# taylor-santos/RelativityPathTracer

Hardware: AMD Instinct MI355X
Metric: Mrays/s (primary rays) on Scenes/bunny.txt at 3840x2160 (higher is better)
Workload: dtype f32

## Files before the change

relativitypathtracer_amd/csrc/rpt_api.hip:

```cpp
#include <hip/hip_runtime.h>

#include <cmath>
#include <cstdio>
#include <chrono>
#include <cstdlib>
#include <cstring>
#include <algorithm>
#include <atomic>
#include <functional>
#include <map>
#include <memory>
#include <mutex>
#include <string>
#include <utility>
#include <vector>

#include "../../include/rpt.h"
#include "rpt_kernels.hip.h"
#include "rpt_octree_build.hip.h"
#include "rpt_screen_bounds.hpp"
#include "rpt_bounds_certify.hpp"
#include "rpt_tile_bitmap.hpp"
#include "rpt_sky_split.hpp"
#include "rpt_workers.hpp"
// ... 909 lines not shown
    a.claim_set = (int)(ctx->claim_epoch++ & 1u);
    unsigned int *claims = (unsigned int *)ctx->claim_counters.ptr;
    const long long want = (band + sky + 3) / 4;
    static const int wgs_per_cu = std::getenv("RPT_WGS_PER_CU") ? std::atoi(std::getenv("RPT_WGS_PER_CU")) : 5;
    const unsigned int wgs = (unsigned int)std::max(1ll, std::min((long long)ctx->cu_count * wgs_per_cu, want));
    switch (v) {
    case 60: hipLaunchKernelGGL(rptd::rpt_render_kernel_persistent_w5, dim3(wgs), dim3(256), 0, ctx->stream, a, a.out16, a.plane, a.debug_rgb, claims); break;
    case 62: hipLaunchKernelGGL(rptd::rpt_render_kernel_persistent_direct_w5, dim3(wgs), dim3(256), 0, ctx->stream, a, a.out16, a.plane, a.debug_rgb, claims); break;
    case 63: hipLaunchKernelGGL(rptd::rpt_render_kernel_persistent_classic_w5, dim3(wgs), dim3(256), 0, ctx->stream, a, a.out16, a.plane, a.debug_rgb, claims); break;
    default: return fail(ctx, RPT_ERR_ARG, "unknown persistent kernel variant");
    }
    return RPT_OK;
}
#endif

#ifdef RPT_DIAGNOSTICS
#define RPT_LAUNCH_X(N) case N: hipLaunchKernelGGL(rptd::rpt_render_kernel_x##N, grid, dim3(256), 0, ctx->stream, a); break;
void launch_sky_fill(rpt_ctx *ctx, const rptd::KernelArgs &a, int tiles, const int box[4]);
int launch_diagnostic(rpt_ctx *ctx, rptd::KernelArgs &a, dim3 grid, int tiles, int v) {
    if (v == 143 || v == 2573 || (v >= 256 && v < 1000 && (v & 8))) set_band_first(ctx, a, tiles);
    switch (v) {
    case 26: {
        const int tiles_x = ((ctx->width + 31) / 32) * 4;
        const int n_tiles = tiles_x * tiles;
        if (int rc = reserve(ctx, ctx->tile_masks, (size_t)n_tiles * 8)) return rc;
        a.mask_tiles_x = tiles_x;
        a.n_tiles = n_tiles;
        a.tile_masks = (unsigned long long *)ctx->tile_masks.ptr;
        hipLaunchKernelGGL(rptd::rpt_tile_bin_kernel, dim3((n_tiles + 255) / 256), dim3(256), 0, ctx->stream, a);
        hipLaunchKernelGGL(rptd::rpt_render_kernel_v1_masked_w5, grid, dim3(256), 0, ctx->stream, a);
        break;
    }
    case 40: hipLaunchKernelGGL(rptd::rpt_render_kernel_ballot_w4, dim3(grid.x * 4, grid.y), dim3(64), 0, ctx->stream, a); break;
    case 42: hipLaunchKernelGGL(rptd::rpt_render_kernel_ballot_w6, dim3(grid.x * 4, grid.y), dim3(64), 0, ctx->stream, a); break;
    case 141: hipLaunchKernelGGL(rptd::rpt_render_kernel_r02walk_w5, grid, dim3(256), 0, ctx->stream, a); break;
    case 143: hipLaunchKernelGGL(rptd::rpt_render_kernel_r02walk_first_w5, grid, dim3(256), 0, ctx->stream, a); break;
    case 60: case 62: case 63: {
        const int rc = launch_persistent(ctx, a, tiles, v);
        if (rc > 0) return rc;
        if (rc < 0) hipLaunchKernelGGL(rptd::rpt_render_kernel_ballot_w5, dim3(grid.x * 4, grid.y), dim3(64), 0, ctx->stream, a);
        break;
    }
    case 61: hipLaunchKernelGGL(rptd::rpt_render_kernel_queue_w5, grid, dim3(256), 0, ctx->stream, a); break;
    RPT_LAUNCH_X(256) RPT_LAUNCH_X(257) RPT_LAUNCH_X(259) RPT_LAUNCH_X(261) RPT_LAUNCH_X(263) RPT_LAUNCH_X(265) RPT_LAUNCH_X(269)
    RPT_LAUNCH_X(273) RPT_LAUNCH_X(277) RPT_LAUNCH_X(285) RPT_LAUNCH_X(305) RPT_LAUNCH_X(317) RPT_LAUNCH_X(337) RPT_LAUNCH_X(349) RPT_LAUNCH_X(401) RPT_LAUNCH_X(785) RPT_LAUNCH_X(529) RPT_LAUNCH_X(541) RPT_LAUNCH_X(561) RPT_LAUNCH_X(573) RPT_LAUNCH_X(621) RPT_LAUNCH_X(641) RPT_LAUNCH_X(653)
    case 1257: hipLaunchKernelGGL(rptd::rpt_render_kernel_x257_w6, grid, dim3(256), 0, ctx->stream, a); break;
    case 2257: hipLaunchKernelGGL(rptd::rpt_render_kernel_x257_w4, grid, dim3(256), 0, ctx->stream, a); break;
    case 2259: hipLaunchKernelGGL(rptd::rpt_render_kernel_x259_w4, grid, dim3(256), 0, ctx->stream, a); break;
    case 2263: hipLaunchKernelGGL(rptd::rpt_render_kernel_x263_w4, grid, dim3(256), 0, ctx->stream, a); break;
    RPT_LAUNCH_X(689) RPT_LAUNCH_X(701)
    case 2573: hipLaunchKernelGGL(rptd::rpt_render_kernel_x573_w4, grid, dim3(256), 0, ctx->stream, a); break;
    case 7:
        if (int rc = reserve(ctx, ctx->counters, 16 * sizeof(unsigned long long))) return rc;
        RPT_HIP(ctx, hipMemsetAsync(ctx->counters.ptr, 0, 16 * sizeof(unsigned long long), ctx->stream));
        a.counters = (unsigned long long *)ctx->counters.ptr;
        hipLaunchKernelGGL(rptd::rpt_render_kernel_v1_diag, grid, dim3(256), 0, ctx->stream, a);
        break;
    case 8: hipLaunchKernelGGL(rptd::rpt_render_kernel_primary_only, grid, dim3(256), 0, ctx->stream, a); break;
    case 786: {
        if (!a.out16) return fail(ctx, RPT_ERR_ARG, "variant 786 writes the 16-byte framebuffer only");
        const int no_box[4] = {0, 0, 0, 0};
        launch_sky_fill(ctx, a, tiles, no_box);
        break;
    }
    case 11:
        if (int rc = reserve(ctx, ctx->wave_times, (size_t)grid.x * grid.y * 4 * 10 * sizeof(unsigned long long))) return rc;
        RPT_HIP(ctx, hipMemsetAsync(ctx->wave_times.ptr, 0, ctx->wave_times.bytes, ctx->stream));
// ... 2819 lines not shown
```

relativitypathtracer_amd/csrc/rpt_diag_kernels.hip.h:

```cpp
#pragma once

namespace rptd {

RPT_DEV f3 cull_dir(const DObj &o, f3 nd) {
    return mk3(o.B[0] * nd.x + o.B[1] * nd.y + o.B[2] * nd.z + o.b[0],
               o.B[3] * nd.x + o.B[4] * nd.y + o.B[5] * nd.z + o.b[1],
               o.B[6] * nd.x + o.B[7] * nd.y + o.B[8] * nd.z + o.b[2]);
}

__global__ __launch_bounds__(256) void rpt_tile_bin_kernel(const KernelArgs a) {
    const int tile = blockIdx.x * 256 + threadIdx.x;
    const bool valid = tile < a.n_tiles;
    unsigned long long mask = 0;
    if (valid) {
        const int tx = tile % a.mask_tiles_x, trow = tile / a.mask_tiles_x;
        const float x0 = (float)(tx * 8);
        const float y0 = (float)(((trow >> a.run_log2) * a.tile_step + a.first_tile + (trow & ((1 << a.run_log2) - 1))) * RPT_TILE_ROWS);
        const float xs[5] = {x0 + 3.5f, x0 - 0.5f, x0 + 7.5f, x0 - 0.5f, x0 + 7.5f};
        const float ys[5] = {y0 + 3.5f, y0 - 0.5f, y0 - 0.5f, y0 + 7.5f, y0 + 7.5f};
        f3 nd[5];
        for (int k = 0; k < 5; k++) {
            const f3 p = mk3((xs[k] / (float)a.width - 0.5f) * a.aspect, ys[k] / (float)a.height - 0.5f, 0.5f);
            nd[k] = p * (1.0f / __builtin_sqrtf(dot(p, p)));
        }
// ... 22 lines not shown
                const float thTile = 1.05f * sTile;
                const f3 to = mk3(o.cbx - o.ox, o.cby - o.oy, o.cbz - o.oz);
                const float dist = __builtin_sqrtf(dot(to, to));
                const bool sane = tile_ok && (sTile < 0.2f) && (lmin > 0.05f * lmax) && (lmax < 1.0e30f) && (dist > 1.05f * o.rb) && (dist < 1.0e30f);
                if (sane) {
                    const f3 ca = cross(u[0], to);
                    const float sinAng = __builtin_sqrtf(dot(ca, ca)) / dist;
                    const float angLow = dot(u[0], to) > 0.0f ? sinAng : 1.0f;
                    const float xs_ = o.rb / dist;
                    const float thObj = xs_ < 0.45f ? 1.05f * xs_ : asinf(fminf(xs_, 1.0f));
                    keep = !(angLow > thObj + 1.5f * thTile + 1.0e-4f);
                }
            }
            if (keep) mask |= 1ull << i;
        }
        if (a.object_count > 64) mask |= 0ull;
        a.tile_masks[tile] = mask;
    }
}


template <int N> struct DiagPolicy : KernelPolicy {
    static constexpr bool culled = N >= 20;
    static constexpr bool band_first = N == 123 || (N >= 256 && N < 1000 && (N & 8));
    static constexpr bool one_wave = false;
    static constexpr int diag = N;
};

__global__ __launch_bounds__(256) void rpt_render_kernel_v1_diag(const KernelArgs a) { render_pixel_body<DiagPolicy<2>>(a); }
__global__ __launch_bounds__(256) __attribute__((amdgpu_waves_per_eu(4, 4))) void rpt_render_kernel_v1_timeline(const KernelArgs a) { render_pixel_body<DiagPolicy<4>>(a); }
__global__ __launch_bounds__(256) void rpt_render_kernel_primary_only(const KernelArgs a) { render_pixel_body<DiagPolicy<5>>(a); }
__global__ __launch_bounds__(256) __attribute__((amdgpu_waves_per_eu(5, 5))) void rpt_render_kernel_v1_masked_w5(const KernelArgs a) { render_pixel_body<DiagPolicy<10>>(a); }
__global__ __launch_bounds__(64) __attribute__((amdgpu_waves_per_eu(4, 4))) void rpt_render_kernel_ballot_w4(const KernelArgs a) { render_pixel_body<Ballot>(a); }
__global__ __launch_bounds__(64) __attribute__((amdgpu_waves_per_eu(6, 6))) void rpt_render_kernel_ballot_w6(const KernelArgs a) { render_pixel_body<Ballot>(a); }
__global__ __launch_bounds__(256) __attribute__((amdgpu_waves_per_eu(5, 5))) void rpt_render_kernel_r02walk_w5(const KernelArgs a) { render_pixel_body<DiagPolicy<120>>(a); }
__global__ __launch_bounds__(256) __attribute__((amdgpu_waves_per_eu(5, 5))) void rpt_render_kernel_r02walk_first_w5(const KernelArgs a) { render_pixel_body<DiagPolicy<123>>(a); }
#define RPT_X_KERNEL(N) __global__ __launch_bounds__(256) __attribute__((amdgpu_waves_per_eu(5, 5))) void rpt_render_kernel_x##N(const KernelArgs a) { render_pixel_body<DiagPolicy<N>>(a); }
#define RPT_XW_KERNEL(N, W) __global__ __launch_bounds__(256) __attribute__((amdgpu_waves_per_eu(W, W))) void rpt_render_kernel_x##N##_w##W(const KernelArgs a) { render_pixel_body<DiagPolicy<N>>(a); }
RPT_XW_KERNEL(257, 6) RPT_XW_KERNEL(257, 4) RPT_XW_KERNEL(263, 4) RPT_XW_KERNEL(259, 4) RPT_XW_KERNEL(573, 4)
RPT_X_KERNEL(256) RPT_X_KERNEL(257) RPT_X_KERNEL(259) RPT_X_KERNEL(261) RPT_X_KERNEL(263) RPT_X_KERNEL(265) RPT_X_KERNEL(269)
RPT_X_KERNEL(273) RPT_X_KERNEL(277) RPT_X_KERNEL(285) RPT_X_KERNEL(305) RPT_X_KERNEL(317) RPT_X_KERNEL(337) RPT_X_KERNEL(349) RPT_X_KERNEL(401) RPT_X_KERNEL(785) RPT_X_KERNEL(529) RPT_X_KERNEL(541) RPT_X_KERNEL(561) RPT_X_KERNEL(573) RPT_X_KERNEL(621) RPT_X_KERNEL(641) RPT_X_KERNEL(653) RPT_X_KERNEL(689) RPT_X_KERNEL(701)

}

#include "rpt_persistent.hip.h"
```

relativitypathtracer_amd/csrc/rpt_kernels.hip.h:

```cpp
#pragma once
#include "../../include/rpt_layout.h"
#include "rpt_device_math.hip.h"

#ifdef RPT_RELAXED_FP
#pragma clang fp contract(fast)
#else
#pragma clang fp contract(off)
#endif

namespace rptd {

#define RPT_EPSILON 0.0000001f
#define RPT_MAX_LEAF_STEPS 4096
#define RPT_LINK_CHILD_MASK 0x00ffffff
#define RPT_TOP_MAX 3072
#define RPT_PI_D 3.14159265358979323846264338327950288

struct alignas(64) DNode {
    float minx, miny, minz; int link;
    float maxx, maxy, maxz; int leafBegin;
    int leafCount; int nb[6]; int pad;
};
static_assert(sizeof(DNode) == 64, "DNode is one 64-B line");
struct alignas(16) DTri { float ax, ay, az, e1x; float e1y, e1z, e2x, e2y; float e2z; int tri; int pad0, pad1; };
// ... 169 lines not shown
RPT_DEV bool intersect_AABB(f3 bmin, f3 bmax, const Ray &ray, f2 &d, int &closeSide, int &farSide) {
    const f3 origin = ray.origin;
    const f3 inv_dir = mk3(1.0f / ray.dir.x, 1.0f / ray.dir.y, 1.0f / ray.dir.z);
    const int sx = inv_dir.x < 0 ? 1 : 0, sy = inv_dir.y < 0 ? 1 : 0, sz = inv_dir.z < 0 ? 1 : 0;
    d.x = ((sx ? bmax.x : bmin.x) - origin.x) * inv_dir.x;
    d.y = ((sx ? bmin.x : bmax.x) - origin.x) * inv_dir.x;
    closeSide = 2 + sx;
    farSide = 3 - sx;
    const float tymin = ((sy ? bmax.y : bmin.y) - origin.y) * inv_dir.y;
    const float tymax = ((sy ? bmin.y : bmax.y) - origin.y) * inv_dir.y;
    if ((d.x > tymax) || (tymin > d.y)) return false;
    if (tymin > d.x) { d.x = tymin; closeSide = 4 + sy; }
    if (tymax < d.y) { d.y = tymax; farSide = 5 - sy; }
    const float tzmin = ((sz ? bmax.z : bmin.z) - origin.z) * inv_dir.z;
    const float tzmax = ((sz ? bmin.z : bmax.z) - origin.z) * inv_dir.z;
    if ((d.x > tzmax) || (tzmin > d.y)) return false;
    if (tzmin > d.x) { d.x = tzmin; closeSide = sz; }
    if (tzmax < d.y) { d.y = tzmax; farSide = 1 - sz; }
    return d.y > 0;
}

struct ExitPlan { f3 scaledDir, inv_dir; int sx, sy, sz; };

RPT_DEV ExitPlan makeExitPlan(f3 scaledDir) {
    ExitPlan p;
    p.scaledDir = scaledDir;
    p.inv_dir = mk3(1.0f / scaledDir.x, 1.0f / scaledDir.y, 1.0f / scaledDir.z);
    p.sx = p.inv_dir.x < 0;
    p.sy = p.inv_dir.y < 0;
    p.sz = p.inv_dir.z < 0;
    return p;
}

RPT_DEV int getOppositeBoxSide(const ExitPlan &p, f3 &uv) {
    const float dx = ((float)(1 - p.sx) - uv.x) * p.inv_dir.x;
    const float dy = ((float)(1 - p.sy) - uv.y) * p.inv_dir.y;
    const float dz = ((float)(1 - p.sz) - uv.z) * p.inv_dir.z;
    float t;
    int side;
    if (dx < dy) {
        if (dx < dz) { t = dx; side = 3 - p.sx; } else { t = dz; side = 1 - p.sz; }
    } else {
        if (dy < dz) { t = dy; side = 5 - p.sy; } else { t = dz; side = 1 - p.sz; }
    }
    uv = uv + p.scaledDir * t;
    return side;
}

RPT_DEV int octree_child_step(f3 &uv);
RPT_DEV int octree_child_step_fast(f3 &uv) {
    const unsigned int lim = 0x3FC00000u;
    const bool in_range = (__float_as_uint(uv.x) < lim) && (__float_as_uint(uv.y) < lim) && (__float_as_uint(uv.z) < lim);
    if (!in_range) return octree_child_step(uv);
    const float top = 1.0f - RPT_EPSILON;
    const bool bx = uv.x >= 0.5f, by = uv.y >= 0.5f, bz = uv.z >= 0.5f;
    const float mx = top < uv.x ? top : uv.x, my = top < uv.y ? top : uv.y, mz = top < uv.z ? top : uv.z;
    uv.x = 2.0f * (mx - (bx ? 0.5f : 0.0f));
    uv.y = 2.0f * (my - (by ? 0.5f : 0.0f));
    uv.z = 2.0f * (mz - (bz ? 0.5f : 0.0f));
    return (bz ? 1 : 0) + (by ? 2 : 0) + (bx ? 4 : 0);
}

RPT_DEV int octree_child_step(f3 &uv) {
    const float fidx = __builtin_roundf(uv.z) + 2 * __builtin_roundf(uv.y) + 4 * __builtin_roundf(uv.x);
    const int childIndex = !(fidx >= 0.0f) ? 0 : (fidx > 7.0f ? 7 : (int)fidx);
    uv.x = 2.0f * fmod_half(cl_min(uv.x, 1.0f - RPT_EPSILON));
// ... 185 lines not shown
        r.tri = 0;
    } else {
        const float2 t2 = *reinterpret_cast<const float2 *>(p + 2);
        r.e2z = t2.x;
        r.tri = __float_as_int(t2.y);
    }
    return r;
}
template <bool EXACT_RCP = false>
RPT_DEV void test_tri_rec(const TriRec &r, const Ray &ray, Hit &hit, int &hitTri, bool &didHit) {
    float dist;
    f2 triUV;
    if (intersect_triangle_edges<EXACT_RCP>(mk3(r.t0.x, r.t0.y, r.t0.z), mk3(r.t0.w, r.t1.x, r.t1.y), mk3(r.t1.z, r.t1.w, r.e2z), ray, dist, triUV)) {
        if (0 <= dist && dist < hit.dist) {
            hitTri = r.tri;
            hit.dist = dist;
            hit.uv = triUV;
            didHit = true;
        }
    }
}

RPT_DEV int descend_to_leaf(const KernelArgs &a, int link, f3 &uv) {
    int idx;
    for (;;) {
        const int k = octree_child_step_fast(uv);
        idx = (link & RPT_LINK_CHILD_MASK) + k;
        if ((link >> (24 + k)) & 1) break;
        link = a.links[idx];
    }
    return idx;
}

template <bool LATENCY, bool EXACT_RCP, bool EXITS = (RPT_EXIT_RECORDS != 0) && !LATENCY>
RPT_DEV bool octree_walk(const KernelArgs &a, const rpt_object &obj, int root, const Ray &newRay, f3 world_origin,
                         float world_dirlen, Hit &hit) {
    static_assert(!(EXITS && LATENCY), "exit records: the throughput walk only");
    int curr = root;
    NodeRec rec = load_node_rec<!LATENCY>(a, curr);
    f2 d;
    int closeSide, farSide;
    f3 nmin = mk3(rec.lo.x, rec.lo.y, rec.lo.z), nmax = mk3(rec.hi.x, rec.hi.y, rec.hi.z);
    if (!intersect_AABB(nmin, nmax, newRay, d, closeSide, farSide)) return false;
    f3 uv = newRay.origin + newRay.dir * d.x;
    if (d.x < 0) {
        uv = (newRay.origin - nmin) / (nmax - nmin);
        if (__float_as_int(rec.lo.w) != -1) {
            curr = descend_to_leaf(a, __float_as_int(rec.lo.w), uv);
            rec = load_node_rec<!LATENCY>(a, curr);
        }
        nmin = mk3(rec.lo.x, rec.lo.y, rec.lo.z);
        nmax = mk3(rec.hi.x, rec.hi.y, rec.hi.z);
        if (!intersect_AABB(nmin, nmax, newRay, d, closeSide, farSide)) return false;
        uv = newRay.origin + newRay.dir * d.x;
    }
    const ExitPlan plan = makeExitPlan(normalize(newRay.dir / (nmax - nmin)));
    bool didHit = false;
    int hitTri = 0;
    TriRec first;
    if (LATENCY) first = load_first_tri<true>(a, curr);
    for (int steps = 1; steps <= RPT_MAX_LEAF_STEPS; steps++) {
        nmin = mk3(rec.lo.x, rec.lo.y, rec.lo.z);
        nmax = mk3(rec.hi.x, rec.hi.y, rec.hi.z);
        uv = (uv - nmin) / (nmax - nmin);
        if (__float_as_int(rec.lo.w) != -1) {
            curr = descend_to_leaf(a, __float_as_int(rec.lo.w), uv);
            rec = load_node_rec<!LATENCY>(a, curr);
            if (LATENCY) first = load_first_tri<true>(a, curr);
            nmin = mk3(rec.lo.x, rec.lo.y, rec.lo.z);
            nmax = mk3(rec.hi.x, rec.hi.y, rec.hi.z);
        }
        int i = __float_as_int(rec.hi.w) & RPT_NODE_BEGIN_MASK;
        const int trisEnd = i + rec.count;
        farSide = getOppositeBoxSide(plan, uv);
        int next = 0;
        if (!EXITS) next = a.dnodes[curr].nb[farSide];
        if (LATENCY) {
            if (i < trisEnd) {
                TriRec cur = first;
                for (; i < trisEnd; i++) {
                    TriRec nxt = cur;
                    if (i + 1 < trisEnd) nxt = load_tri_rec<true>(a, i + 1);
                    cur.tri = i;
                    test_tri_rec<EXACT_RCP>(cur, newRay, hit, hitTri, didHit);
                    cur = nxt;
                }
            }
        } else {
            for (; i < trisEnd; i++) test_tri_rec<EXACT_RCP>(load_tri_rec<true>(a, i), newRay, hit, hitTri, didHit);
// ... 24 lines not shown
    return true;
}

#ifdef RPT_DIAGNOSTICS
}
#include "rpt_diag_walks.hip.h"
namespace rptd {
#endif

enum class Walk {
    reference,
    none,
    throughput,
    latency,
};
enum class Camera {
    pinhole,
    equirect,
    lens,
    raymap,
};
struct KernelPolicy {
    static constexpr Walk walk = Walk::throughput;
    static constexpr Camera camera = Camera::pinhole;
    static constexpr bool exact_rcp = false;
    static constexpr bool culled = true;
    static constexpr bool object_mask = true;
    static constexpr bool tile_bits = true;
    static constexpr bool band_first = false;
    static constexpr bool one_wave = true;
    static constexpr bool doppler = false;
    static constexpr bool drec = false;
    static constexpr bool environment = false;
    static constexpr bool windowed = false;
    static constexpr int diag = 0;
};
struct RefLayout : KernelPolicy { static constexpr Walk walk = Walk::reference; static constexpr bool culled = false; };
struct Unculled : KernelPolicy { static constexpr bool culled = false; };
struct Ballot : KernelPolicy {};
struct BallotExact : Ballot { static constexpr bool exact_rcp = true; };
struct BallotFirst : KernelPolicy { static constexpr Walk walk = Walk::latency; static constexpr bool band_first = true; };
struct BallotFirstExact : BallotFirst { static constexpr bool exact_rcp = true; };
struct Analytic : KernelPolicy { static constexpr Walk walk = Walk::none; static constexpr bool tile_bits = false; };
template <class P> struct DopplerTwin : P { static constexpr bool doppler = true; };
struct DopplerRecorded : DopplerTwin<Unculled> { static constexpr bool drec = true; };
template <class P> struct Panorama : P { static constexpr Camera camera = Camera::equirect; static constexpr bool object_mask = false; };
struct PanoramaWalk : Panorama<BallotExact> {};
struct PanoramaWalkIeee : Panorama<Ballot> {};
struct PanoramaAnalytic : Panorama<Analytic> {};
struct PanoramaUnculled : Panorama<Unculled> {};
struct PanoramaRecorded : Panorama<DopplerRecorded> {};
template <class P> struct Environment : DopplerTwin<P> { static constexpr bool environment = true; };
template <class P> struct Lens : P { static constexpr Camera camera = Camera::lens; };
template <class P> struct Raymap : P { static constexpr Camera camera = Camera::raymap; static constexpr bool object_mask = false; static constexpr bool tile_bits = false; };

template <class P> struct Windowed : P { static constexpr bool windowed = true; };

#ifdef RPT_RELAXED_FP
template <class P> constexpr bool tile_origin_policy = false;
#else
template <class P> constexpr bool tile_origin_policy = P::one_wave && P::culled && P::object_mask && P::camera == Camera::pinhole && !P::doppler && !P::environment && !P::windowed && !P::band_first && P::diag == 0;
#endif

RPT_DEV bool window_accepts(const DObj &pre, float t) { return !(t < pre.win_t0) && !(t >= pre.win_t1); }

template <class P>
RPT_DEV bool mesh_walk(const KernelArgs &a, const rpt_object &obj, int i, const Ray &newRay, f3 world_origin, float world_dirlen, Hit &hit) {
#ifdef RPT_DIAGNOSTICS
    if constexpr (P::diag != 0) return diag_walk<P::diag>(a, obj, a.dobjs[i].root, newRay, world_origin, world_dirlen, hit);
#endif
    if (P::walk == Walk::reference) return octree_core_ref(a, obj, newRay, world_origin, world_dirlen, hit);
    return octree_walk<P::walk == Walk::latency, P::exact_rcp>(a, obj, a.dobjs[i].root, newRay, world_origin, world_dirlen, hit);
}

RPT_DEV float max3(f3 v) { return cl_max(cl_max(v.x, v.y), v.z); }
RPT_DEV float cube_winding(f3 origin) {
    return max3(mk3(__builtin_fabsf(origin.x), __builtin_fabsf(origin.y), __builtin_fabsf(origin.z))) < 1.0f ? -1.0f : 1.0f;
}

RPT_DEV bool cube_core(const rpt_object &obj, f3 origin, float winding, f3 dir, float scale, Hit &hit) {
    f3 sgn = mk3(-cl_sign(dir.x), -cl_sign(dir.y), -cl_sign(dir.z));
    const f3 d = (sgn * winding - origin) / dir;
#define RPT_TEST(U, V, W) ((d.U >= 0.0f) && (__builtin_fabsf(origin.V + dir.V * d.U) < 1.0f) && (__builtin_fabsf(origin.W + dir.W * d.U) < 1.0f))
    if (RPT_TEST(x, y, z)) sgn = mk3(sgn.x, 0, 0);
    else if (RPT_TEST(y, z, x)) sgn = mk3(0, sgn.y, 0);
    else sgn = mk3(0, 0, RPT_TEST(z, x, y) ? sgn.z : 0);
#undef RPT_TEST
    const bool any = (sgn.x != 0) || (sgn.y != 0) || (sgn.z != 0);
    if (!any) return false;
    const float dist = (sgn.x != 0) ? d.x : ((sgn.y != 0) ? d.y : d.z);
    const f3 objPt = origin + dir * dist;
    hit.dist = dist / scale;
    hit.normal = normalize(applyTranspose(obj.InvM, sgn));
    if (sgn.x != 0) { hit.uv.x = (objPt.y + 1) / 2; hit.uv.y = (objPt.z + 1) / 2; }
    else if (sgn.y != 0) { hit.uv.x = (objPt.x + 1) / 2; hit.uv.y = (objPt.z + 1) / 2; }
    else { hit.uv.x = (objPt.x + 1) / 2; hit.uv.y = (objPt.y + 1) / 2; }
    return true;
}

RPT_DEV bool sphere_core(const rpt_object &obj, f3 rayToSphere, float c, f3 dir, float scale, Hit &hit, bool want_uv) {
    const float b = dot(rayToSphere, dir);
    float disc = b * b - c;
    if (disc < 0.0f) return false;
    disc = __builtin_sqrtf(disc);
    float dist;
// ... 121 lines not shown
    addr = addr < 0 ? 0 : addr;
    addr = addr >= a.texture_bytes ? a.texture_bytes - 1 : addr;
    return a.textures[addr] / 255.0f;
}
RPT_DEV f3 texel3(const KernelArgs &a, int offset, int width, int x, int y) {
    const long long base = (long long)offset + 3 * ((long long)width * y + x);
    return mk3(texel(a, base + 0), texel(a, base + 1), texel(a, base + 2));
}

RPT_DEV f3 sample_texture(const KernelArgs &a, const rpt_object &ho, f2 huv) {
    const int width = ho.textureWidth;
    const int height = ho.textureHeight;
    const float u = width * huv.x;
    const float v = height * (1.0f - huv.y);
    int x = imin(f2i_sat(__builtin_floorf(u)), width - 1);
    int y = imin(f2i_sat(__builtin_floorf(v)), height - 1);
    const float u_ratio = u - x;
    const float v_ratio = v - y;
    const float u_opp = 1 - u_ratio;
    const float v_opp = 1 - v_ratio;
    const int offset = ho.textureIndex;
    f3 result = texel3(a, offset, width, x, y) * u_opp;
    x = iclamp(x + 1, 0, width - 1);
    result = result + texel3(a, offset, width, x, y) * u_ratio;
    result = result * v_opp;
    y = iclamp(y + 1, 0, height - 1);
    f3 result2 = texel3(a, offset, width, x, y) * u_ratio;
    x = iclamp(x - 1, 0, width - 1);
    result2 = result2 + texel3(a, offset, width, x, y) * u_opp;
    result2 = result2 * v_ratio;
    return result + result2;
}

template <class P>
RPT_DEV bool sample_light_occluded(const KernelArgs &a, f4 origin4, f4 dir4, float lightDist, int lightIndex) {
    const f3 nd = normalize(yzw(dir4));
    const f4 lightDir0 = mk4((float)a.interval, nd.x, nd.y, nd.z);
    for (int i = 0; i < a.object_count; i++) {
        if (i != lightIndex) {
            Hit newHit;
            newHit.dist = 1e20f;
            const f4 newEvent0 = transformPoint4D(a.objects[i].Lorentz, origin4);
            const f4 lightDir = transformPoint4D(a.objects[i].Lorentz, lightDir0);
            if (intersect_object<P>(a, i, newEvent0, lightDir, newHit, lightDist)) {
                if constexpr (P::windowed) {
                    if (newHit.dist < lightDist && window_accepts(a.dobjs[i], newEvent0.x + lightDir.x * newHit.dist)) return true;
                } else {
                    if (newHit.dist < lightDist) return true;
                }
            }
        }
    }
    return false;
}

#define RPT_DOPPLER_RECORD 11
#define RPT_NU_R ((float)(546.1 / 700.0))
#define RPT_NU_B ((float)(546.1 / 435.8))
#define RPT_NU_K0 ((float)(2.0 * (546.1 / 700.0) - 1.0))
#define RPT_NU_K4 ((float)(2.0 * (546.1 / 435.8) - 1.0))

RPT_DEV float doppler_spectrum(float u, float r, float g, float b) {
    if (!(u > RPT_NU_K0) || !(u < RPT_NU_K4)) return 0.0f;
    float xa, xb, ya, yb;
    if (u < RPT_NU_R) { xa = RPT_NU_K0; xb = RPT_NU_R; ya = 0.0f; yb = r; }
    else if (u < 1.0f) { xa = RPT_NU_R; xb = 1.0f; ya = r; yb = g; }
// ... 38 lines not shown
    int x = iclamp(f2i_sat(__builtin_floorf(u)), 0, width - 1);
    int y = iclamp(f2i_sat(__builtin_floorf(v)), 0, height - 1);
    const float u_ratio = u - x;
    const float v_ratio = v - y;
    const float u_opp = 1 - u_ratio;
    const float v_opp = 1 - v_ratio;
    f3 result = environment_texel(texels, width, x, y) * u_opp;
    x = x + 1 >= width ? 0 : x + 1;
    result = result + environment_texel(texels, width, x, y) * u_ratio;
    result = result * v_opp;
    y = iclamp(y + 1, 0, height - 1);
    f3 result2 = environment_texel(texels, width, x, y) * u_ratio;
    x = x - 1 < 0 ? width - 1 : x - 1;
    result2 = result2 + environment_texel(texels, width, x, y) * u_opp;
    result2 = result2 * v_ratio;
    return result + result2;
}
RPT_DEV f3 environment_colour(const EnvironmentArgs &a, f3 camdir) {
    const f3 nd = normalize(camdir);
    const f4 rayDir = mk4((float)a.interval, nd.x, nd.y, nd.z);
    const f4 k = transformPoint4D(a.env_frame, rayDir);
    const f3 d = normalize(yzw(k));
    f3 c = environment_bilinear(a.env_texels, a.env_width, a.env_height, environment_uv(d));
    if (a.doppler != 0 && a.interval != 0) c = doppler_colour(a.doppler, (float)a.interval / k.x, c);
    return c;
}

struct DopplerRecord {
    float dcam, dlight;
    f3 ref, lit;
};

template <class P>
RPT_DEV bool trace(const KernelArgs &a, f3 camdir, unsigned long long object_mask, f3 &color_out, DopplerRecord *rec = nullptr) {
    const float inf = 1e20f;
    Hit hit;
    hit.dist = inf;
    hit.object = -1;
    const f3 nd = normalize(camdir);
    const f4 rayDir = mk4((float)a.interval, nd.x, nd.y, nd.z);

    for (int i = 0; i < a.object_count; i++) {
        if (i < 64 && !((object_mask >> i) & 1ull)) continue;
        Hit newHit;
        newHit.dist = inf;
        bool got;
        if (P::walk == Walk::reference) got = intersect_object<P>(a, i, ld4(a.objects[i].stationaryCam), transformPoint4D(a.objects[i].Lorentz, rayDir), newHit);
        else got = intersect_object_primary<P>(a, i, rayDir, newHit);
        if (got) {
            if constexpr (P::windowed) {
                if (newHit.dist < hit.dist && window_accepts(a.dobjs[i], a.objects[i].stationaryCam.x + dot(ld4(a.objects[i].Lorentz[0]), rayDir) * newHit.dist)) {
                    hit = newHit;
                    hit.object = i;
                }
            } else if (newHit.dist < hit.dist) {
                hit = newHit;
                hit.object = i;
            }
        }
    }
    if (hit.object < 0) return false;
#ifdef RPT_DIAGNOSTICS
    if (P::diag == 5) {
        color_out = mk3(hit.dist, hit.normal.x + hit.uv.x, hit.normal.y + hit.normal.z + hit.uv.y);
        return true;
    }
#endif

    const rpt_object &ho = a.objects[hit.object];
    f3 hcolor = ho.textureIndex != -1 ? sample_texture(a, ho, hit.uv) : ld3(ho.color);
    if (ho.flashPeriod > 0) {
        const float event_x = ho.stationaryCam.x + dot(ld4(ho.Lorentz[0]), rayDir) * hit.dist;
        const float period = ho.flashPeriod;
        const float duration = ho.flashDuration;
        if (event_x - period * __builtin_floorf(event_x / period) < duration) hcolor = hcolor * 2;
    }

    f3 color = hcolor * (a.interval != 0 ? a.ambient : 1.0f);
    if (ho.light) color = color + hcolor;
    [[maybe_unused]] f3 color_ref = color;
    [[maybe_unused]] float dlight = 1.0f;
    [[maybe_unused]] bool lit_any = false;
    if (a.interval != 0) {
        for (int i = 0; i < a.object_count; i++) {
            if (i != hit.object && a.objects[i].light) {
                const rpt_object &lo = a.objects[i];
                const f4 cameraPos_ObjFrame = ld4(ho.stationaryCam);
                const f4 rayDir_ObjFrame = transformPoint4D(ho.Lorentz, rayDir);
                f4 hitPos_ObjFrame = cameraPos_ObjFrame + rayDir_ObjFrame * hit.dist;
                hitPos_ObjFrame = hitPos_ObjFrame + mk4(0, hit.normal.x * 0.001f, hit.normal.y * 0.001f, hit.normal.z * 0.001f);
                const f4 hitPos = transformPoint4D(ho.InvLorentz, hitPos_ObjFrame);
                const f4 hitPos_LightFrame = transformPoint4D(lo.Lorentz, hitPos);
                const f3 lightPos3_LightFrame = mk3(lo.M[0].w, lo.M[1].w, lo.M[2].w);
                const f3 lightDir3_LightFrame = lightPos3_LightFrame - yzw(hitPos_LightFrame);
                const f4 lightDir_LightFrame = mk4(a.interval * length(lightDir3_LightFrame), lightDir3_LightFrame.x,
                                                   lightDir3_LightFrame.y, lightDir3_LightFrame.z);
                if constexpr (P::windowed) {
                    if (!window_accepts(a.dobjs[i], hitPos_LightFrame.x + lightDir_LightFrame.x)) continue;
                }
                const f4 lightDir = transformPoint4D(lo.InvLorentz, lightDir_LightFrame);
                const f4 lightDir_ObjFrame = transformPoint4D(ho.Lorentz, lightDir);
                const f3 lightDir3_ObjFrame = yzw(lightDir_ObjFrame);
                const f3 unitLightDir3 = normalize(lightDir3_ObjFrame);
                const float ndotl = dot(hit.normal, unitLightDir3);
                if (ndotl > 0) {
                    const f3 ld = normalize(yzw(lightDir));
                    const f4 shadowDir = mk4((float)a.interval, ld.x, ld.y, ld.z);
                    if (!sample_light_occluded<P>(a, hitPos, shadowDir, length(yzw(lightDir)), i)) {
                        const float k = ndotl / (1.0f + 0.1f * length(lightDir3_ObjFrame) +
                                                 0.01f * dot(lightDir3_ObjFrame, lightDir3_ObjFrame));
                        if constexpr (P::doppler) {
                            const float di = lightDir_ObjFrame.x / lightDir_LightFrame.x;
                            if constexpr (P::drec) {
                                color_ref = color_ref + hcolor * k * ld3(lo.color);
                                if (!lit_any) dlight = di;
                                lit_any = true;
// ... 333 lines not shown
        const f4 rayDir = mk4((float)a.interval, nd.x, nd.y, nd.z);
        for (int i = 0; i < a.object_count; i++) {
            if (i < 64 && !((object_mask >> i) & 1ull)) continue;
            Hit newHit;
            newHit.dist = inf;
            if (intersect_object_primary<P>(a, i, rayDir, newHit)) {
                if constexpr (P::windowed) {
                    if (newHit.dist < hit.dist && window_accepts(a.dobjs[i], a.objects[i].stationaryCam.x + dot(ld4(a.objects[i].Lorentz[0]), rayDir) * newHit.dist)) {
                        hit = newHit;
                        hit.object = i;
                    }
                } else if (newHit.dist < hit.dist) {
                    hit = newHit;
                    hit.object = i;
                }
            }
        }
        if (hit.object >= 0) {
            const rpt_object &ho = a.objects[hit.object];
            if (ho.type == RPT_SPHERE && ho.textureIndex == -1) hit.uv = primary_sphere_uv(a, hit.object, rayDir);
            const f4 lightDir = transformPoint4D(ho.Lorentz, rayDir);
            ev = ld4(ho.stationaryCam) + lightDir * hit.dist;
            object = hit.object;
            dist = hit.dist;
            uv = hit.uv;
        }
    }
    store_event(a.events, (size_t)y_coord * a.width + x_coord, object, dist, ev, uv);
}

#ifndef RPT_RELAXED_FP
__global__ __launch_bounds__(64) void rpt_render_kernel_v0(const KernelArgs a) { render_pixel_body<RefLayout>(a); }
__global__ __launch_bounds__(64) __attribute__((amdgpu_waves_per_eu(5, 5))) void rpt_render_kernel_unculled_w5(const KernelArgs a) { render_pixel_body<Unculled>(a); }
__global__ __launch_bounds__(64) __attribute__((amdgpu_waves_per_eu(5, 5))) void rpt_render_kernel_ballot_w5(const KernelArgs a) { render_pixel_body<BallotExact>(a); }
__global__ __launch_bounds__(64) __attribute__((amdgpu_waves_per_eu(5, 5))) void rpt_render_kernel_ballot_first_w5(const KernelArgs a) { render_pixel_body<BallotFirstExact>(a); }
__global__ __launch_bounds__(64) __attribute__((amdgpu_waves_per_eu(5, 5))) void rpt_render_kernel_ballot_ieee_w5(const KernelArgs a) { render_pixel_body<Ballot>(a); }
__global__ __launch_bounds__(64) __attribute__((amdgpu_waves_per_eu(5, 5))) void rpt_render_kernel_ballot_first_ieee_w5(const KernelArgs a) { render_pixel_body<BallotFirst>(a); }
__global__ __launch_bounds__(64) __attribute__((amdgpu_waves_per_eu(8, 8))) void rpt_render_kernel_analytic_w8(const KernelArgs a) { render_pixel_body<Analytic>(a); }

#define RPT_SKY_FILL_TILES 8
struct SkyFillArgs {
    rpt_pixel *out16;
    int width, height;
    uint32_t bg_packed;
    int tx0, ty0, tx1, ty1;
};
__global__ __launch_bounds__(64) __attribute__((amdgpu_waves_per_eu(8, 8))) void rpt_sky_fill_kernel(const SkyFillArgs a) {
    const int lane = threadIdx.x & 63;
    const int ty = (int)blockIdx.y, tx_first = (int)blockIdx.x * RPT_SKY_FILL_TILES;
    const bool box_rows = ty >= a.ty0 && ty < a.ty1;
    if (box_rows && tx_first >= a.tx0 && tx_first + RPT_SKY_FILL_TILES <= a.tx1) return;
    const int y = ty * RPT_TILE_ROWS + (lane >> 3);
    if (y >= a.height) return;
    const uint32_t fy = __float_as_uint((float)y);
    const size_t row = (size_t)y * a.width;
#pragma unroll
    for (int k = 0; k < RPT_SKY_FILL_TILES; k++) {
        const int tx = tx_first + k, x = tx * 8 + (lane & 7);
        const bool in_box = box_rows && tx >= a.tx0 && tx < a.tx1;
        if (!in_box && x < a.width) store_pixel(a.out16, row + x, __float_as_uint((float)x), fy, a.bg_packed, 0u);
    }
}

__global__ __launch_bounds__(64) __attribute__((amdgpu_waves_per_eu(5, 5))) void rpt_render_kernel_msaa_w5(const KernelArgs a) { render_pixel_body_msaa<Ballot>(a); }
__global__ __launch_bounds__(64) __attribute__((amdgpu_waves_per_eu(5, 5))) void rpt_render_kernel_msaa_unculled_w5(const KernelArgs a) { render_pixel_body_msaa<Unculled>(a); }

__global__ __launch_bounds__(64) __attribute__((amdgpu_waves_per_eu(5, 5))) void rpt_render_kernel_unculled_doppler_w5(const DopplerArgs a) { render_pixel_body<DopplerTwin<Unculled>>(a); }
__global__ __launch_bounds__(64) __attribute__((amdgpu_waves_per_eu(5, 5))) void rpt_render_kernel_ballot_doppler_w5(const DopplerArgs a) { render_pixel_body<DopplerTwin<BallotExact>>(a); }
__global__ __launch_bounds__(64) __attribute__((amdgpu_waves_per_eu(5, 5))) void rpt_render_kernel_ballot_first_doppler_w5(const DopplerArgs a) { render_pixel_body<DopplerTwin<BallotFirstExact>>(a); }
// ... 775 lines not shown
```

Baseline: 122,700.

## Park shading state in LDS during shadow rays to raise ballot kernel occupancy

Adds a parked variant of the light loop that stores hit color, normal, distance, direction and object id in per-lane LDS slots while shadow rays are traced, reloading them afterwards. This lowers live VGPRs across the occluder walk. The main ballot kernels now request 6 waves per EU instead of 5. The octree walk also gets a compact exit plan that packs far-side signs into a bitmask to save registers. Extra LDS traffic and volatile accesses are the cost, and the static_assert requiring one_wave may not hold for these policies.

```diff
diff --git a/relativitypathtracer_amd/csrc/rpt_api.hip b/relativitypathtracer_amd/csrc/rpt_api.hip
--- a/relativitypathtracer_amd/csrc/rpt_api.hip
+++ b/relativitypathtracer_amd/csrc/rpt_api.hip
@@ -965,7 +965,10 @@
         break;
     }
     case 40: hipLaunchKernelGGL(rptd::rpt_render_kernel_ballot_w4, dim3(grid.x * 4, grid.y), dim3(64), 0, ctx->stream, a); break;
-    case 42: hipLaunchKernelGGL(rptd::rpt_render_kernel_ballot_w6, dim3(grid.x * 4, grid.y), dim3(64), 0, ctx->stream, a); break;
+    case 42:
+        if (ctx->geo->exact_rcp_ok) hipLaunchKernelGGL(rptd::rpt_render_kernel_ballot_w6, dim3(grid.x * 4, grid.y), dim3(64), 0, ctx->stream, a);
+        else hipLaunchKernelGGL(rptd::rpt_render_kernel_ballot_ieee_w6, dim3(grid.x * 4, grid.y), dim3(64), 0, ctx->stream, a);
+        break;
     case 141: hipLaunchKernelGGL(rptd::rpt_render_kernel_r02walk_w5, grid, dim3(256), 0, ctx->stream, a); break;
     case 143: hipLaunchKernelGGL(rptd::rpt_render_kernel_r02walk_first_w5, grid, dim3(256), 0, ctx->stream, a); break;
     case 60: case 62: case 63: {
diff --git a/relativitypathtracer_amd/csrc/rpt_diag_kernels.hip.h b/relativitypathtracer_amd/csrc/rpt_diag_kernels.hip.h
--- a/relativitypathtracer_amd/csrc/rpt_diag_kernels.hip.h
+++ b/relativitypathtracer_amd/csrc/rpt_diag_kernels.hip.h
@@ -78,7 +78,8 @@
 __global__ __launch_bounds__(256) void rpt_render_kernel_primary_only(const KernelArgs a) { render_pixel_body<DiagPolicy<5>>(a); }
 __global__ __launch_bounds__(256) __attribute__((amdgpu_waves_per_eu(5, 5))) void rpt_render_kernel_v1_masked_w5(const KernelArgs a) { render_pixel_body<DiagPolicy<10>>(a); }
 __global__ __launch_bounds__(64) __attribute__((amdgpu_waves_per_eu(4, 4))) void rpt_render_kernel_ballot_w4(const KernelArgs a) { render_pixel_body<Ballot>(a); }
-__global__ __launch_bounds__(64) __attribute__((amdgpu_waves_per_eu(6, 6))) void rpt_render_kernel_ballot_w6(const KernelArgs a) { render_pixel_body<Ballot>(a); }
+__global__ __launch_bounds__(64) __attribute__((amdgpu_waves_per_eu(6, 6))) void rpt_render_kernel_ballot_w6(const KernelArgs a) { render_pixel_body<BallotExact>(a); }
+__global__ __launch_bounds__(64) __attribute__((amdgpu_waves_per_eu(6, 6))) void rpt_render_kernel_ballot_ieee_w6(const KernelArgs a) { render_pixel_body<Ballot>(a); }
 __global__ __launch_bounds__(256) __attribute__((amdgpu_waves_per_eu(5, 5))) void rpt_render_kernel_r02walk_w5(const KernelArgs a) { render_pixel_body<DiagPolicy<120>>(a); }
 __global__ __launch_bounds__(256) __attribute__((amdgpu_waves_per_eu(5, 5))) void rpt_render_kernel_r02walk_first_w5(const KernelArgs a) { render_pixel_body<DiagPolicy<123>>(a); }
 #define RPT_X_KERNEL(N) __global__ __launch_bounds__(256) __attribute__((amdgpu_waves_per_eu(5, 5))) void rpt_render_kernel_x##N(const KernelArgs a) { render_pixel_body<DiagPolicy<N>>(a); }
diff --git a/relativitypathtracer_amd/csrc/rpt_kernels.hip.h b/relativitypathtracer_amd/csrc/rpt_kernels.hip.h
--- a/relativitypathtracer_amd/csrc/rpt_kernels.hip.h
+++ b/relativitypathtracer_amd/csrc/rpt_kernels.hip.h
@@ -225,6 +225,33 @@
     return p;
 }
 
+struct ExitPlanBits { f3 scaledDir, inv_dir; int far_bits; };
+
+RPT_DEV ExitPlanBits makeExitPlanBits(f3 scaledDir) {
+    const ExitPlan q = makeExitPlan(scaledDir);
+    ExitPlanBits p;
+    p.scaledDir = q.scaledDir;
+    p.inv_dir = q.inv_dir;
+    p.far_bits = (1 - q.sx) | ((1 - q.sy) << 1) | ((1 - q.sz) << 2);
+    return p;
+}
+
+RPT_DEV int getOppositeBoxSide(const ExitPlanBits &p, f3 &uv) {
+    const int bx = p.far_bits & 1, by = (p.far_bits >> 1) & 1, bz = p.far_bits >> 2;
+    const float dx = ((float)bx - uv.x) * p.inv_dir.x;
+    const float dy = ((float)by - uv.y) * p.inv_dir.y;
+    const float dz = ((float)bz - uv.z) * p.inv_dir.z;
+    float t;
+    int first, place;
+    if (dx < dy) {
+        if (dx < dz) { t = dx; first = 2; place = 0; } else { t = dz; first = 0; place = 2; }
+    } else {
+        if (dy < dz) { t = dy; first = 4; place = 1; } else { t = dz; first = 0; place = 2; }
+    }
+    uv = uv + p.scaledDir * t;
+    return first + ((p.far_bits >> place) & 1);
+}
+
 RPT_DEV int getOppositeBoxSide(const ExitPlan &p, f3 &uv) {
     const float dx = ((float)(1 - p.sx) - uv.x) * p.inv_dir.x;
     const float dy = ((float)(1 - p.sy) - uv.y) * p.inv_dir.y;
@@ -476,10 +503,11 @@
     return idx;
 }
 
-template <bool LATENCY, bool EXACT_RCP, bool EXITS = (RPT_EXIT_RECORDS != 0) && !LATENCY>
+template <bool LATENCY, bool EXACT_RCP, bool FACE_BITS = false, bool EXITS = (RPT_EXIT_RECORDS != 0) && !LATENCY>
 RPT_DEV bool octree_walk(const KernelArgs &a, const rpt_object &obj, int root, const Ray &newRay, f3 world_origin,
                          float world_dirlen, Hit &hit) {
     static_assert(!(EXITS && LATENCY), "exit records: the throughput walk only");
+    static_assert(!(FACE_BITS && LATENCY), "the latency walk keeps its plan");
     int curr = root;
     NodeRec rec = load_node_rec<!LATENCY>(a, curr);
     f2 d;
@@ -498,7 +526,8 @@
         if (!intersect_AABB(nmin, nmax, newRay, d, closeSide, farSide)) return false;
         uv = newRay.origin + newRay.dir * d.x;
     }
-    const ExitPlan plan = makeExitPlan(normalize(newRay.dir / (nmax - nmin)));
+    const f3 planDir = normalize(newRay.dir / (nmax - nmin));
+    const auto plan = [&] { if constexpr (FACE_BITS) return makeExitPlanBits(planDir); else return makeExitPlan(planDir); }();
     bool didHit = false;
     int hitTri = 0;
     TriRec first;
@@ -589,6 +618,7 @@
     static constexpr bool doppler = false;
     static constexpr bool drec = false;
     static constexpr bool environment = false;
+    static constexpr bool park_bystanders = false;
     static constexpr bool windowed = false;
     static constexpr int diag = 0;
 };
@@ -596,6 +626,8 @@
 struct Unculled : KernelPolicy { static constexpr bool culled = false; };
 struct Ballot : KernelPolicy {};
 struct BallotExact : Ballot { static constexpr bool exact_rcp = true; };
+struct BallotExactParked : BallotExact { static constexpr bool park_bystanders = true; };
+struct BallotParked : Ballot { static constexpr bool park_bystanders = true; };
 struct BallotFirst : KernelPolicy { static constexpr Walk walk = Walk::latency; static constexpr bool band_first = true; };
 struct BallotFirstExact : BallotFirst { static constexpr bool exact_rcp = true; };
 struct Analytic : KernelPolicy { static constexpr Walk walk = Walk::none; static constexpr bool tile_bits = false; };
@@ -627,7 +659,7 @@
     if constexpr (P::diag != 0) return diag_walk<P::diag>(a, obj, a.dobjs[i].root, newRay, world_origin, world_dirlen, hit);
 #endif
     if (P::walk == Walk::reference) return octree_core_ref(a, obj, newRay, world_origin, world_dirlen, hit);
-    return octree_walk<P::walk == Walk::latency, P::exact_rcp>(a, obj, a.dobjs[i].root, newRay, world_origin, world_dirlen, hit);
+    return octree_walk<P::walk == Walk::latency, P::exact_rcp, P::park_bystanders && P::walk == Walk::throughput>(a, obj, a.dobjs[i].root, newRay, world_origin, world_dirlen, hit);
 }
 
 RPT_DEV float max3(f3 v) { return cl_max(cl_max(v.x, v.y), v.z); }
@@ -815,6 +847,23 @@
     return result + result2;
 }
 
+#define RPT_PARK_SLOTS 17
+enum ParkSlot {
+    PARK_HCOLOR = 0,
+    PARK_COLOR = 3,
+    PARK_NORMAL = 6,
+    PARK_DIST = 9,
+    PARK_ND = 10,
+    PARK_OBJECT = 13,
+    PARK_L3 = 14,
+};
+__shared__ float park_lds[RPT_PARK_SLOTS][64];
+typedef volatile __attribute__((address_space(3))) float park_word;
+RPT_DEV void park_put(int k, float v) { *(park_word *)&park_lds[k][threadIdx.x & 63] = v; }
+RPT_DEV float park_get(int k) { return *(park_word *)&park_lds[k][threadIdx.x & 63]; }
+RPT_DEV void park_put3(int k, f3 v) { park_put(k, v.x); park_put(k + 1, v.y); park_put(k + 2, v.z); }
+RPT_DEV f3 park_get3(int k) { const float x = park_get(k), y = park_get(k + 1), z = park_get(k + 2); return mk3(x, y, z); }
+
 template <class P>
 RPT_DEV bool sample_light_occluded(const KernelArgs &a, f4 origin4, f4 dir4, float lightDist, int lightIndex) {
     const f3 nd = normalize(yzw(dir4));
@@ -919,6 +968,52 @@
 };
 
 template <class P>
+RPT_DEV f3 trace_lights_parked(const KernelArgs &a, f3 nd, const Hit &hit, f3 hcolor, f3 color) {
+    static_assert(!P::doppler && !P::windowed && !P::drec && P::one_wave, "parking: kernel 41's policy only");
+    park_put3(PARK_HCOLOR, hcolor);
+    park_put3(PARK_COLOR, color);
+    park_put3(PARK_NORMAL, hit.normal);
+    park_put(PARK_DIST, hit.dist);
+    park_put3(PARK_ND, nd);
+    park_put(PARK_OBJECT, __int_as_float(hit.object));
+    for (int i = 0; i < a.object_count; i++) {
+        const int object = __float_as_int(park_get(PARK_OBJECT));
+        if (i != object && a.objects[i].light) {
+            const rpt_object &ho = a.objects[object];
+            const rpt_object &lo = a.objects[i];
+            const f3 normal = park_get3(PARK_NORMAL), d3 = park_get3(PARK_ND);
+            const f4 rayDir = mk4((float)a.interval, d3.x, d3.y, d3.z);
+            const f4 cameraPos_ObjFrame = ld4(ho.stationaryCam);
+            const f4 rayDir_ObjFrame = transformPoint4D(ho.Lorentz, rayDir);
+            f4 hitPos_ObjFrame = cameraPos_ObjFrame + rayDir_ObjFrame * park_get(PARK_DIST);
+            hitPos_ObjFrame = hitPos_ObjFrame + mk4(0, normal.x * 0.001f, normal.y * 0.001f, normal.z * 0.001f);
+            const f4 hitPos = transformPoint4D(ho.InvLorentz, hitPos_ObjFrame);
+            const f4 hitPos_LightFrame = transformPoint4D(lo.Lorentz, hitPos);
+            const f3 lightPos3_LightFrame = mk3(lo.M[0].w, lo.M[1].w, lo.M[2].w);
+            const f3 lightDir3_LightFrame = lightPos3_LightFrame - yzw(hitPos_LightFrame);
+            const f4 lightDir_LightFrame = mk4(a.interval * length(lightDir3_LightFrame), lightDir3_LightFrame.x,
+                                               lightDir3_LightFrame.y, lightDir3_LightFrame.z);
+            const f4 lightDir = transformPoint4D(lo.InvLorentz, lightDir_LightFrame);
+            const f4 lightDir_ObjFrame = transformPoint4D(ho.Lorentz, lightDir);
+            const f3 lightDir3_ObjFrame = yzw(lightDir_ObjFrame);
+            if (dot(normal, normalize(lightDir3_ObjFrame)) > 0) {
+                park_put3(PARK_L3, lightDir3_ObjFrame);
+                const f3 ld = normalize(yzw(lightDir));
+                const f4 shadowDir = mk4((float)a.interval, ld.x, ld.y, ld.z);
+                if (!sample_light_occluded<P>(a, hitPos, shadowDir, length(yzw(lightDir)), i)) {
+                    const f3 l3 = park_get3(PARK_L3);
+                    const float ndotl = dot(park_get3(PARK_NORMAL), normalize(l3));
+                    const float k = ndotl / (1.0f + 0.1f * length(l3) + 0.01f * dot(l3, l3));
+                    const f3 sum = park_get3(PARK_COLOR) + park_get3(PARK_HCOLOR) * k * ld3(lo.color);
+                    park_put3(PARK_COLOR, sum);
+                }
+            }
+        }
+    }
+    return park_get3(PARK_COLOR);
+}
+
+template <class P>
 RPT_DEV bool trace(const KernelArgs &a, f3 camdir, unsigned long long object_mask, f3 &color_out, DopplerRecord *rec = nullptr) {
     const float inf = 1e20f;
     Hit hit;
@@ -968,7 +1063,9 @@
     [[maybe_unused]] f3 color_ref = color;
     [[maybe_unused]] float dlight = 1.0f;
     [[maybe_unused]] bool lit_any = false;
-    if (a.interval != 0) {
+    if constexpr (P::park_bystanders) {
+        if (a.interval != 0) color = trace_lights_parked<P>(a, nd, hit, hcolor, color);
+    } else if (a.interval != 0) {
         for (int i = 0; i < a.object_count; i++) {
             if (i != hit.object && a.objects[i].light) {
                 const rpt_object &lo = a.objects[i];
@@ -1368,9 +1465,9 @@
 #ifndef RPT_RELAXED_FP
 __global__ __launch_bounds__(64) void rpt_render_kernel_v0(const KernelArgs a) { render_pixel_body<RefLayout>(a); }
 __global__ __launch_bounds__(64) __attribute__((amdgpu_waves_per_eu(5, 5))) void rpt_render_kernel_unculled_w5(const KernelArgs a) { render_pixel_body<Unculled>(a); }
-__global__ __launch_bounds__(64) __attribute__((amdgpu_waves_per_eu(5, 5))) void rpt_render_kernel_ballot_w5(const KernelArgs a) { render_pixel_body<BallotExact>(a); }
+__global__ __launch_bounds__(64) __attribute__((amdgpu_waves_per_eu(6, 6))) void rpt_render_kernel_ballot_w5(const KernelArgs a) { render_pixel_body<BallotExactParked>(a); }
 __global__ __launch_bounds__(64) __attribute__((amdgpu_waves_per_eu(5, 5))) void rpt_render_kernel_ballot_first_w5(const KernelArgs a) { render_pixel_body<BallotFirstExact>(a); }
-__global__ __launch_bounds__(64) __attribute__((amdgpu_waves_per_eu(5, 5))) void rpt_render_kernel_ballot_ieee_w5(const KernelArgs a) { render_pixel_body<Ballot>(a); }
+__global__ __launch_bounds__(64) __attribute__((amdgpu_waves_per_eu(6, 6))) void rpt_render_kernel_ballot_ieee_w5(const KernelArgs a) { render_pixel_body<BallotParked>(a); }
 __global__ __launch_bounds__(64) __attribute__((amdgpu_waves_per_eu(5, 5))) void rpt_render_kernel_ballot_first_ieee_w5(const KernelArgs a) { render_pixel_body<BallotFirst>(a); }
 __global__ __launch_bounds__(64) __attribute__((amdgpu_waves_per_eu(8, 8))) void rpt_render_kernel_analytic_w8(const KernelArgs a) { render_pixel_body<Analytic>(a); }
 
```

Result: faster. 134,200, median of 6 (+9.4%).
